# XuyangBai/D3Feat

Hardware: NVIDIA H100
Metric: points/sec through KPFCNN encoder (higher is better)
Workload: dtype f32

## Files before the change

### d3feat_b200/csrc/pool.cu

```cuda
#include "ops.cuh"

namespace d3f {

__global__ void __launch_bounds__(256) colmin_kernel(const float* __restrict__ x, int Ncap, const int* __restrict__ n_dev,
                                                     int C, unsigned* __restrict__ colmin_ord) {
  const int N = dyn_rows(Ncap, n_dev);
  __shared__ unsigned red[8][32];
  if (colmin_ord[C] != 0u) return;
  const int tx = threadIdx.x & 31, ty = threadIdx.x >> 5;
  const int c = blockIdx.x * 32 + tx;
  unsigned m = 0xffffffffu;
  if (c < C)
    for (int r = blockIdx.y * 8 + ty; r < N; r += gridDim.y * 8) m = min(m, f2ord(x[(size_t)r * C + c]));
  red[ty][tx] = m;
  __syncthreads();
  if (ty == 0 && c < C) {
#pragma unroll
    for (int k = 1; k < 8; ++k) m = min(m, red[k][tx]);
    atomicMin(&colmin_ord[c], m);
  }
}

template <int VEC>
__global__ void __launch_bounds__(256)
ind_max_pool_kernel(const float* __restrict__ x, const int* __restrict__ inds, int N1cap, int N2cap,
                    const int* __restrict__ n1_dev, const int* __restrict__ n2_dev, int H, int C, int slabs,
                    unsigned* __restrict__ colmin_ord, float* __restrict__ out) {
  const int N1 = dyn_rows(N1cap, n1_dev), N2 = dyn_rows(N2cap, n2_dev);
  const int gw = (blockIdx.x * blockDim.x + threadIdx.x) >> 5, lane = threadIdx.x & 31;
  const int warp = gw / slabs, slab = gw - warp * slabs;
  if (warp >= N2) return;
  const int* row = inds + (size_t)warp * H;
  const int c0 = slab * 32 * VEC + lane * VEC;
  if (c0 >= C) return;
  float best[VEC];
#pragma unroll
  for (int v = 0; v < VEC; ++v) best[v] = -3.402823466e38f;
  bool any_real = false;
  for (int h = 0; h < H; ++h) {
    int id = row[h];
    if (id < 0 || id >= N1) continue;
    any_real = true;
    const float* p = x + (size_t)id * C + c0;
    if (VEC == 4) {
      float4 t = *reinterpret_cast<const float4*>(p);
      best[0] = fmaxf(best[0], t.x); best[1 % VEC] = fmaxf(best[1 % VEC], t.y);
      best[2 % VEC] = fmaxf(best[2 % VEC], t.z); best[3 % VEC] = fmaxf(best[3 % VEC], t.w);
    } else {
      best[0] = fmaxf(best[0], *p);
    }
  }
  if (!any_real) {
    if (lane == 0 && slab == 0) colmin_ord[C] = 0u;
    return;
  }
  if (VEC == 4) {
    *reinterpret_cast<float4*>(out + (size_t)warp * C + c0) =
        make_float4(best[0], best[1 % VEC], best[2 % VEC], best[3 % VEC]);
  } else {
    out[(size_t)warp * C + c0] = best[0];
  }
}

__global__ void __launch_bounds__(256)
ind_max_pool_fix_kernel(const int* __restrict__ inds, int N1cap, int N2cap, const int* __restrict__ n1_dev,
                        const int* __restrict__ n2_dev, int H, int C, const unsigned* __restrict__ colmin_ord,
                        float* __restrict__ out) {
  if (colmin_ord[C] != 0u) return;
  const int N1 = dyn_rows(N1cap, n1_dev), N2 = dyn_rows(N2cap, n2_dev);
  const int lane = threadIdx.x & 31;
  for (int r = (blockIdx.x * blockDim.x + threadIdx.x) >> 5; r < N2; r += (gridDim.x * blockDim.x) >> 5) {
    bool real = false;
    for (int h = lane; h < H; h += 32) {
      int id = inds[(size_t)r * H + h];
      real = real || (id >= 0 && id < N1);
    }
    if (__any_sync(0xffffffffu, real)) continue;
    for (int c = lane; c < C; c += 32) out[(size_t)r * C + c] = ord2f(colmin_ord[c]);
  }
}

int ind_max_pool(const float* x, const int* inds, int N1, int N2, int H, int C, float* out, void* workspace,
                 size_t workspace_bytes, cudaStream_t stream, const int* n1_dev, const int* n2_dev) {
  D3F_REQUIRE(N1 >= 1 && N2 >= 0 && H >= 0 && C >= 1, D3F_ERR_INVALID, "ind_max_pool: bad shape N1=%d N2=%d H=%d C=%d",
              N1, N2, H, C);
  D3F_REQUIRE(workspace_bytes >= sizeof(unsigned) * ((size_t)C + 1), D3F_ERR_WORKSPACE,
              "ind_max_pool: workspace too small");
  if (N2 == 0) return D3F_OK;
  unsigned* colmin = (unsigned*)workspace;
  D3F_CUDA(cudaMemsetAsync(colmin, 0xff, sizeof(unsigned) * ((size_t)C + 1), stream));
  int blocks = ceil_div(N2 * 32, 256);
  bool v4 = (C % 4 == 0) && ((reinterpret_cast<uintptr_t>(x) & 15) == 0) && ((reinterpret_cast<uintptr_t>(out) & 15) == 0);
  const int slabs = ceil_div(C, v4 ? 128 : 32);
  const long long pool_blocks = ((long long)N2 * slabs * 32 + 255) / 256;
  D3F_REQUIRE(pool_blocks < (1ll << 31), D3F_ERR_CAPACITY, "ind_max_pool: %d rows x %d channels exceed the launch grid", N2, C);
  if (v4) ind_max_pool_kernel<4><<<(unsigned)pool_blocks, 256, 0, stream>>>(x, inds, N1, N2, n1_dev, n2_dev, H, C, slabs, colmin, out);
  else ind_max_pool_kernel<1><<<(unsigned)pool_blocks, 256, 0, stream>>>(x, inds, N1, N2, n1_dev, n2_dev, H, C, slabs, colmin, out);
  D3F_LAUNCH_CHECK("ind_max_pool_kernel");
  dim3 grid(ceil_div(C, 32), min(ceil_div(N1, 64), 4 * kNumSMs));
  colmin_kernel<<<grid, 256, 0, stream>>>(x, N1, n1_dev, C, colmin);
  D3F_LAUNCH_CHECK("colmin_kernel");
  ind_max_pool_fix_kernel<<<min(blocks, 4 * kNumSMs), 256, 0, stream>>>(inds, N1, N2, n1_dev, n2_dev, H, C, colmin, out);
  D3F_LAUNCH_CHECK("ind_max_pool_fix_kernel");
  return D3F_OK;
}

__global__ void __launch_bounds__(256)
closest_pool_kernel(const float* __restrict__ x, const int* __restrict__ inds, int N1cap, int N2cap,
                    const int* __restrict__ n1_dev, const int* __restrict__ n2_dev, int ld, int C,
                    float* __restrict__ out) {
  const int N1 = dyn_rows(N1cap, n1_dev), N2 = dyn_rows(N2cap, n2_dev);
  const int warp = (blockIdx.x * blockDim.x + threadIdx.x) >> 5, lane = threadIdx.x & 31;
  if (warp >= N2) return;
  int id = inds[(size_t)warp * ld];
  bool shadow = id < 0 || id >= N1;
  for (int c = lane; c < C; c += 32) out[(size_t)warp * C + c] = shadow ? 0.f : x[(size_t)id * C + c];
}

int closest_pool(const float* x, const int* inds, int N1, int N2, int ld_inds, int C, float* out, cudaStream_t stream,
                 const int* n1_dev, const int* n2_dev) {
  D3F_REQUIRE(N1 >= 0 && N2 >= 0 && ld_inds >= 1 && C >= 1, D3F_ERR_INVALID, "closest_pool: bad shape");
  if (N2 == 0) return D3F_OK;
  closest_pool_kernel<<<ceil_div(N2 * 32, 256), 256, 0, stream>>>(x, inds, N1, N2, n1_dev, n2_dev, ld_inds, C, out);
  D3F_LAUNCH_CHECK("closest_pool_kernel");
  return D3F_OK;
}

__global__ void __launch_bounds__(256) l2_normalize_kernel(const float* __restrict__ x, int Ncap,
                                                           const int* __restrict__ n_dev, int C, float eps,
                                                           float* __restrict__ out) {
  const int N = dyn_rows(Ncap, n_dev);
  const int warp = (blockIdx.x * blockDim.x + threadIdx.x) >> 5, lane = threadIdx.x & 31;
  if (warp >= N) return;
  float s = 0.f;
  for (int c = lane; c < C; c += 32) {
    float v = x[(size_t)warp * C + c];
    s = fmaf(v, v, s);
  }
#pragma unroll
  for (int o = 16; o > 0; o >>= 1) s += __shfl_xor_sync(0xffffffffu, s, o);
  float inv = rsqrtf(fmaxf(s, eps));
  float m = fmaxf(s, eps);
  inv = inv * (1.5f - 0.5f * m * inv * inv);
  for (int c = lane; c < C; c += 32) out[(size_t)warp * C + c] = x[(size_t)warp * C + c] * inv;
}

int l2_normalize(const float* x, int N, int C, float eps, float* out, cudaStream_t stream, const int* n_dev) {
  D3F_REQUIRE(N >= 0 && C >= 1, D3F_ERR_INVALID, "l2_normalize: bad shape");
  if (N == 0) return D3F_OK;
  l2_normalize_kernel<<<ceil_div(N * 32, 256), 256, 0, stream>>>(x, N, n_dev, C, eps, out);
  D3F_LAUNCH_CHECK("l2_normalize_kernel");
  return D3F_OK;
}

__global__ void __launch_bounds__(256)
cloud_max_kernel(const float* __restrict__ x, int Ncap, const int* __restrict__ n_dev, int D,
                 const int* __restrict__ start, int B, unsigned* __restrict__ cloud_max_ord,
                 unsigned char* __restrict__ nonzero) {
  const int N = dyn_rows(Ncap, n_dev);
  const int warp = (blockIdx.x * blockDim.x + threadIdx.x) >> 5, lane = threadIdx.x & 31;
  if (warp >= N) return;
  float m = -3.402823466e38f, s = 0.f;
  for (int c = lane; c < D; c += 32) {
    float v = x[(size_t)warp * D + c];
    m = fmaxf(m, v);
    s += v;
  }
#pragma unroll
  for (int o = 16; o > 0; o >>= 1) {
    m = fmaxf(m, __shfl_xor_sync(0xffffffffu, m, o));
    s += __shfl_xor_sync(0xffffffffu, s, o);
  }
  if (lane == 0) {
    if (warp < start[B]) atomicMax(&cloud_max_ord[batch_of(start, B, warp)], f2ord(m));
    nonzero[warp] = s != 0.f ? 1 : 0;
  }
}

__global__ void __launch_bounds__(256)
detection_score_kernel(const float* __restrict__ x, const int* __restrict__ nb, int Ncap,
                       const int* __restrict__ n_dev, int H, int D, const int* __restrict__ start, int B,
                       const unsigned* __restrict__ cloud_max_ord, const unsigned char* __restrict__ nonzero,
                       float* __restrict__ score) {
  const int N = dyn_rows(Ncap, n_dev);
  const int warp = (blockIdx.x * blockDim.x + threadIdx.x) >> 5, lane = threadIdx.x & 31;
  if (warp >= N) return;
  const float inv = warp < start[B] ? 1.f / (ord2f(cloud_max_ord[batch_of(start, B, warp)]) + 1e-6f) : 0.f;
  const int* row = nb + (size_t)warp * H;
  int cnt = 0;
  for (int h = 0; h < H; ++h) {
    int id = row[h];
    if (id >= 0 && id < N && nonzero[id]) ++cnt;
  }
  const float inv_cnt = 1.f / (float)max(cnt, 1);
  float dmax = -3.402823466e38f;
  for (int c = lane; c < D; c += 32) dmax = fmaxf(dmax, x[(size_t)warp * D + c] * inv);
#pragma unroll
  for (int o = 16; o > 0; o >>= 1) dmax = fmaxf(dmax, __shfl_xor_sync(0xffffffffu, dmax, o));
  float best = -3.402823466e38f;
  for (int c = lane; c < D; c += 32) {
    const float f = x[(size_t)warp * D + c] * inv;
    float mean = 0.f;
    for (int h = 0; h < H; ++h) {
      int id = row[h];
      if (id >= 0 && id < N) mean += x[(size_t)id * D + c] * inv;
    }
    mean *= inv_cnt;
    const float d = f - mean;
    const float softplus = d > 20.f ? d : log1pf(expf(d));
    best = fmaxf(best, softplus * (f / (1e-6f + dmax)));
  }
#pragma unroll
  for (int o = 16; o > 0; o >>= 1) best = fmaxf(best, __shfl_xor_sync(0xffffffffu, best, o));
  if (lane == 0) score[warp] = best;
}

size_t detection_scores_workspace_bytes(int N, int B) {
  return align_up(sizeof(int) * (size_t)(B + 1), 256) + align_up(sizeof(unsigned) * (size_t)B, 256) + align_up((size_t)N + 1, 256);
}

int detection_scores(const float* feats, const int* neighbors, const int* lengths, int B, int N, int H, int D,
                     float* out_scores, void* workspace, size_t workspace_bytes, cudaStream_t stream,
                     const int* n_dev) {
  D3F_REQUIRE(B >= 1 && B <= kMaxBatch && N >= 0 && H >= 0 && D >= 1, D3F_ERR_INVALID, "detection_scores: bad shape");
  D3F_REQUIRE(workspace_bytes >= detection_scores_workspace_bytes(N, B), D3F_ERR_WORKSPACE, "detection_scores: workspace too small");
  if (N == 0) return D3F_OK;
  Carver cv(workspace, workspace_bytes);
  int* start = cv.take<int>(B + 1);
  unsigned* cmax = cv.take<unsigned>(B);
  unsigned char* nonzero = cv.take<unsigned char>((size_t)N + 1);
  int rc = launch_batch_start(lengths, B, start, stream);
  if (rc) return rc;
  D3F_CUDA(cudaMemsetAsync(cmax, 0, sizeof(unsigned) * B, stream));
  cloud_max_kernel<<<ceil_div(N * 32, 256), 256, 0, stream>>>(feats, N, n_dev, D, start, B, cmax, nonzero);
  D3F_LAUNCH_CHECK("cloud_max_kernel");
  detection_score_kernel<<<ceil_div(N * 32, 256), 256, 0, stream>>>(feats, neighbors, N, n_dev, H, D, start, B, cmax, nonzero, out_scores);
  D3F_LAUNCH_CHECK("detection_score_kernel");
  return D3F_OK;
}

__global__ void __launch_bounds__(256)
affine_leaky_kernel(const float* __restrict__ x, long long total_cap, const int* __restrict__ n_dev, int C,
                    const float* __restrict__ scale, const float* __restrict__ shift,
                    const float* __restrict__ residual, float alpha, float* __restrict__ out) {
  const long long total = n_dev ? min(total_cap, (long long)max(__ldg(n_dev), 0) * C) : total_cap;
  for (long long i = (long long)blockIdx.x * blockDim.x + threadIdx.x; i < total; i += (long long)gridDim.x * blockDim.x) {
    int c = (int)(i % C);
    float y = x[i];
    if (scale) y = fmaf(y, scale[c], shift[c]);
    if (residual) y += residual[i];
    if (alpha >= 0.f) y = y > 0.f ? y : y * alpha;
    out[i] = y;
  }
}

int affine_leaky(const float* x, int N, int C, const float* scale, const float* shift, const float* residual,
                 float alpha, float* out, cudaStream_t stream, const int* n_dev) {
  D3F_REQUIRE(N >= 0 && C >= 1 && (scale == nullptr) == (shift == nullptr), D3F_ERR_INVALID, "affine_leaky: bad arguments");
  long long total = (long long)N * C;
  if (total == 0) return D3F_OK;
  int blocks = (int)min((total + 255) / 256, (long long)kNumSMs * 16);
  affine_leaky_kernel<<<blocks, 256, 0, stream>>>(x, total, n_dev, C, scale, shift, residual, alpha, out);
  D3F_LAUNCH_CHECK("affine_leaky_kernel");
  return D3F_OK;
}

}
```

### d3feat_b200/csrc/tc_gemm.cu

```cuda
#include <cuda.h>
#include <cudaTypedefs.h>
#include <stdlib.h>

#include "ops.cuh"
#include "tc_common.cuh"

namespace d3f {

constexpr int kTcBM = 128;
constexpr int kTcBK = 32;
constexpr int kTcConsumerWarps = 8;
constexpr int kTcThreads = 32 * kTcConsumerWarps + 32;

__global__ void __launch_bounds__(256) pack_weight_kernel(const float* __restrict__ W, int K, int N, int Kpad,
                                                          int Npad, float* __restrict__ packed) {
  long long total = (long long)Npad * Kpad;
  for (long long i = (long long)blockIdx.x * blockDim.x + threadIdx.x; i < total; i += (long long)gridDim.x * blockDim.x) {
    int k = (int)(i / Npad), n = (int)(i % Npad);
    float x = (n < N && k < K) ? W[(size_t)k * N + n] : 0.f;
    float hi, lo;
    split_tf32(x, hi, lo);
    int kc = k >> 5, kl = k & 31;
    size_t slab = (size_t)kc * 2 * Npad * 32;
    size_t off = (size_t)n * 32 + (size_t)((((kl >> 2) ^ (n & 7)) << 2) | (kl & 3));
    packed[slab + off] = hi;
    packed[slab + (size_t)Npad * 32 + off] = lo;
  }
}

int tc_padded_k(int K) { return (K + kTcBK - 1) / kTcBK * kTcBK; }
int tc_block_n(int N) { return N > 64 ? 128 : (N > 32 ? 64 : 32); }
int tc_padded_n(int N) { int bn = tc_block_n(N); return (N + bn - 1) / bn * bn; }
size_t tc_packed_floats(int K, int N) { return 2 * (size_t)tc_padded_k(K) * tc_padded_n(N); }

int tc_pack_weight(const float* W, int K, int N, float* packed, cudaStream_t stream) {
  D3F_REQUIRE(K >= 1 && N >= 1 && W && packed, D3F_ERR_INVALID, "pack_weight: bad arguments");
  int Kpad = tc_padded_k(K), Npad = tc_padded_n(N);
  long long total = (long long)Npad * Kpad;
  int blocks = (int)min((total + 255) / 256, (long long)kNumSMs * 8);
  pack_weight_kernel<<<blocks, 256, 0, stream>>>(W, K, N, Kpad, Npad, packed);
  D3F_LAUNCH_CHECK("pack_weight_kernel");
  return D3F_OK;
}

template <int BN>
struct TcSmem {
  static constexpr int kCtasPerSm = BN >= 128 ? 1 : 2;
  static constexpr int kStages = BN >= 64 ? 3 : 4;
  static constexpr int kABytes = kTcBM * 128;
  static constexpr int kBBytes = BN * 128;
  static constexpr int kStageBytes = kABytes + 2 * kBBytes;
  static constexpr int kEpiWarpBytes = 1024 + 3 * BN * 4;
  static constexpr int kTotal = kStages * kStageBytes + 1024  + 256  + kTcConsumerWarps * kEpiWarpBytes;
  static_assert(kCtasPerSm * (kTotal + 1024) <= 233472, "shared memory of an H100 SM (228 KB, 1 KB reserved per CTA)");
};

template <int BN>
__global__ void __launch_bounds__(kTcThreads, TcSmem<BN>::kCtasPerSm)
tc_gemm_kernel(const __grid_constant__ CUtensorMap tmA, const __grid_constant__ CUtensorMap tmA2, int K1,
               const float* __restrict__ Bp, float* __restrict__ C, int Mcap, int N, int Kpad, int Npad,
               int chunks_per_split, Epilogue ep) {
  const int M = ep.m_dev ? min(Mcap, max(__ldg(ep.m_dev) - ep.m_off, 0)) : Mcap;
  const int ntn = Npad / BN;
  const int tiles = ceil_div(M, kTcBM) * ntn;
  if ((int)blockIdx.x >= tiles) return;
  extern __shared__ uint8_t smem_raw[];
  using S = TcSmem<BN>;
  constexpr int kStages = S::kStages;
  uint8_t* smem = (uint8_t*)(((uintptr_t)smem_raw + 1023) & ~(uintptr_t)1023);
  uint64_t* full = (uint64_t*)(smem + kStages * S::kStageBytes);
  uint64_t* empty = full + kStages;

  const int tid = threadIdx.x, warp = tid >> 5, lane = tid & 31;
  const int kt0 = blockIdx.z * chunks_per_split;
  const int nk = min(Kpad / kTcBK - kt0, chunks_per_split);
  float* Cz = C + (size_t)blockIdx.z * Mcap * N;

  if (tid == 0) {
    for (int s = 0; s < kStages; ++s) {
      mbar_init(smem_u32(&full[s]), 1);
      mbar_init(smem_u32(&empty[s]), kTcConsumerWarps);
    }
    asm volatile("fence.mbarrier_init.release.cluster;" ::: "memory");
  }
  __syncthreads();

  if (warp == kTcConsumerWarps) {
    if (lane == 0) {
      const int total = (tiles - (int)blockIdx.x + (int)gridDim.x - 1) / (int)gridDim.x * nk;
      int tile = (int)blockIdx.x, kt = 0;
      for (int g = 0; g < total; ++g) {
        const int s = g % kStages;
        mbar_wait(smem_u32(&empty[s]), ((uint32_t)(g / kStages) & 1u) ^ 1u);
        const uint32_t st = smem_u32(smem + s * S::kStageBytes);
        const uint32_t fb = smem_u32(&full[s]);
        const int m0 = (tile / ntn) * kTcBM, n0 = (tile % ntn) * BN;
        const int k0 = (kt0 + kt) * kTcBK;
        mbar_arrive_expect_tx(fb, (uint32_t)S::kStageBytes);
        if (k0 < K1)
          tma_load_2d(st, &tmA, k0, m0, fb);
        else
          tma_load_2d(st, &tmA2, k0 - K1, m0, fb);
        const float* slab = Bp + (size_t)(kt0 + kt) * 2 * Npad * 32 + (size_t)n0 * 32;
        tma_bulk_g2s(st + S::kABytes, slab, S::kBBytes, fb);
        tma_bulk_g2s(st + S::kABytes + S::kBBytes, slab + (size_t)Npad * 32, S::kBBytes, fb);
        if (++kt == nk) {
          kt = 0;
          tile += (int)gridDim.x;
        }
      }
    }
  } else {
    constexpr int R = BN / 2;
    const int cw = warp >> 2;
    const int wq = warp & 3;
    const int r0 = 64 * cw + 16 * wq + (lane >> 2);
    const uint32_t a_row = (uint32_t)r0 * 128u + (uint32_t)(lane & 3) * 4u, a_swz = (uint32_t)(r0 & 7);
    auto load_a = [&](float* x, uint32_t sa, int j) {
#pragma unroll
      for (int q = 0; q < 4; ++q)
        x[q] = lds32(sa + a_row + (uint32_t)(q & 1) * 1024u + ((((uint32_t)(2 * j + (q >> 1))) ^ a_swz) << 4));
    };
    float acc[R], sum[R];
    int g = 0;
    for (int t = (int)blockIdx.x; t < tiles; t += (int)gridDim.x) {
      const int m0 = (t / ntn) * kTcBM, n0 = (t % ntn) * BN;
#pragma unroll
      for (int j = 0; j < R; ++j) sum[j] = 0.f;
      for (int kt = 0; kt < nk; ++kt, ++g) {
        const int s = g % kStages;
        mbar_wait(smem_u32(&full[s]), (uint32_t)(g / kStages) & 1u);
        const uint32_t sa = smem_u32(smem + s * S::kStageBytes);
        const uint64_t b_hi = make_smem_desc(sa + S::kABytes), b_lo = make_smem_desc(sa + S::kABytes + S::kBBytes);
        float x[4];
        uint32_t ah[2][4], al[2][4];
        load_a(x, sa, 0);
#pragma unroll
        for (int j = 0; j < R; ++j) acc[j] = 0.f;
#pragma unroll
        for (int j = 0; j < kTcBK / 8; ++j) {
          uint32_t* h = ah[j & 1];
          uint32_t* l = al[j & 1];
#pragma unroll
          for (int q = 0; q < 4; ++q) {
            float hi, lo;
            split_tf32(x[q], hi, lo);
            h[q] = __float_as_uint(hi);
            l[q] = __float_as_uint(lo);
          }
          const uint64_t adv = (uint64_t)((j * 32) >> 4);
          wgmma_fence();
          wgmma_tf32_rs<BN>(acc, h, b_hi + adv);
          wgmma_tf32_rs<BN>(acc, l, b_hi + adv);
          wgmma_tf32_rs<BN>(acc, h, b_lo + adv);
          wgmma_commit();
          if (j + 1 < kTcBK / 8) load_a(x, sa, j + 1);
          wgmma_wait<1>();
        }
        wgmma_wait<0>();
        wgmma_reg_fence<R>(acc);
        __syncwarp();
        if (lane == 0) mbar_arrive(smem_u32(&empty[s]));
#pragma unroll
        for (int j = 0; j < R; ++j) sum[j] += acc[j];
      }
      const bool has_bn = ep.bn_scale != nullptr, has_bias = ep.bias != nullptr, has_res = ep.residual != nullptr;
      const bool has_leaky = ep.leaky_alpha >= 0.f;
      const bool vec = (N & 3) == 0 &&
                       ((reinterpret_cast<uintptr_t>(C) | reinterpret_cast<uintptr_t>(ep.residual)) & 15) == 0;
      const uint32_t st_tile = smem_u32(smem + kStages * S::kStageBytes + 256) + (uint32_t)warp * S::kEpiWarpBytes;
      const uint32_t st_par = st_tile + 1024u;
      if (t == (int)blockIdx.x || ntn > 1) {
        for (int c = lane; c < BN; c += 32) {
          const int n = n0 + c;
          if (has_bn) {
            sts32(st_par + 4u * c, n < N ? ep.bn_scale[n] : 0.f);
            sts32(st_par + 4u * (BN + c), n < N ? ep.bn_shift[n] : 0.f);
          }
          if (has_bias) sts32(st_par + 4u * (2 * BN + c), n < N ? ep.bias[n] : 0.f);
        }
      }
#pragma unroll
      for (int h = 0; h < 2; ++h) {
#pragma unroll
        for (int cg = 0; cg < BN / 32; ++cg) {
          {
            const uint32_t r = (uint32_t)(lane >> 2), tq = (uint32_t)(lane & 3);
            const uint32_t swz = ((r & 3u) << 1) ^ (r >> 2);
#pragma unroll
            for (int jj = 0; jj < 4; ++jj) {
              const int j = 4 * cg + jj;
              sts64(st_tile + r * 128u + (((uint32_t)(2 * jj) + (tq >> 1)) ^ swz) * 16u + (tq & 1u) * 8u,
                    sum[4 * j + 2 * h], sum[4 * j + 2 * h + 1]);
            }
          }
          __syncwarp();
          const int pc = lane & 7;
          const int gn = n0 + 32 * cg + 4 * pc;
          const uint32_t par = st_par + 4u * (32 * cg + 4 * pc);
#pragma unroll
          for (int i = 0; i < 2; ++i) {
            const uint32_t r = (uint32_t)(lane >> 3) + 4u * i;
            const float4 v = lds128(st_tile + r * 128u + (((uint32_t)pc ^ ((r & 3u) << 1) ^ (r >> 2)) << 4));
            const int gm = m0 + 64 * cw + 16 * wq + 8 * h + (int)r;
            if (gm >= M || gn >= N) continue;
            const float rs = ep.rowscale != nullptr ? ep.rowscale[gm] : 1.f;
            const size_t orow = ep.row_map ? (size_t)ep.row_map[gm] : (size_t)gm;
            float* cp = Cz + orow * N + gn;
            const float* rp = has_res ? ep.residual + orow * N + gn : nullptr;
            float y[4] = {v.x * rs, v.y * rs, v.z * rs, v.w * rs};
            float res[4] = {0.f, 0.f, 0.f, 0.f};
            if (has_res) {
              if (vec) {
                const float4 rv = *reinterpret_cast<const float4*>(rp);
                res[0] = rv.x; res[1] = rv.y; res[2] = rv.z; res[3] = rv.w;
              } else {
#pragma unroll
                for (int e = 0; e < 4; ++e)
                  if (gn + e < N) res[e] = rp[e];
              }
            }
            if (has_bn) {
              const float4 sc = lds128(par), sh = lds128(par + 4u * BN);
              y[0] = fmaf(y[0], sc.x, sh.x); y[1] = fmaf(y[1], sc.y, sh.y);
              y[2] = fmaf(y[2], sc.z, sh.z); y[3] = fmaf(y[3], sc.w, sh.w);
            }
            if (has_bias) {
              const float4 bi = lds128(par + 8u * BN);
              y[0] += bi.x; y[1] += bi.y; y[2] += bi.z; y[3] += bi.w;
            }
#pragma unroll
            for (int e = 0; e < 4; ++e) {
              y[e] += res[e];
              if (has_leaky) y[e] = y[e] > 0.f ? y[e] : y[e] * ep.leaky_alpha;
            }
            if (vec) {
              *reinterpret_cast<float4*>(cp) = make_float4(y[0], y[1], y[2], y[3]);
            } else {
#pragma unroll
              for (int e = 0; e < 4; ++e)
                if (gn + e < N) cp[e] = y[e];
            }
          }
          __syncwarp();
        }
      }
    }
  }
}

__global__ void __launch_bounds__(256) splitk_reduce_kernel(const float* __restrict__ part, int splits, int Mcap, int N,
                                                            Epilogue ep, float* __restrict__ C) {
  const int M = ep.m_dev ? min(Mcap, max(__ldg(ep.m_dev) - ep.m_off, 0)) : Mcap;
  const long long slab = (long long)Mcap * N;
  long long total = (long long)M * N;
  for (long long i = (long long)blockIdx.x * blockDim.x + threadIdx.x; i < total; i += (long long)gridDim.x * blockDim.x) {
    int m = (int)(i / N), n = (int)(i % N);
    float y = 0.f;
    for (int z = 0; z < splits; ++z) y += part[(size_t)z * slab + i];
    if (ep.rowscale) y *= ep.rowscale[m];
    if (ep.bn_scale) y = fmaf(y, ep.bn_scale[n], ep.bn_shift[n]);
    if (ep.bias) y += ep.bias[n];
    const size_t orow = ep.row_map ? (size_t)ep.row_map[m] : (size_t)m;
    if (ep.residual) y += ep.residual[orow * N + n];
    if (ep.leaky_alpha >= 0.f) y = y > 0.f ? y : y * ep.leaky_alpha;
    C[orow * N + n] = y;
  }
}

static int encode_a_map(CUtensorMap* map, const float* A, int rows, int cols) {
  static PFN_cuTensorMapEncodeTiled_v12000 encode = nullptr;
  if (encode == nullptr) {
    void* fn = nullptr;
    cudaDriverEntryPointQueryResult q;
    D3F_CUDA(cudaGetDriverEntryPoint("cuTensorMapEncodeTiled", &fn, cudaEnableDefault, &q));
    D3F_REQUIRE(q == cudaDriverEntryPointSuccess && fn != nullptr, D3F_ERR_CUDA,
                "tc_gemm: the driver has no cuTensorMapEncodeTiled");
    encode = reinterpret_cast<PFN_cuTensorMapEncodeTiled_v12000>(fn);
  }
  const cuuint64_t dims[2] = {(cuuint64_t)cols, (cuuint64_t)rows};
  const cuuint64_t strides[1] = {(cuuint64_t)cols * sizeof(float)};
  const cuuint32_t box[2] = {(cuuint32_t)kTcBK, (cuuint32_t)kTcBM};
  const cuuint32_t elem[2] = {1, 1};
  const CUresult r = encode(map, CU_TENSOR_MAP_DATA_TYPE_FLOAT32, 2, const_cast<float*>(A), dims, strides, box, elem,
                            CU_TENSOR_MAP_INTERLEAVE_NONE, CU_TENSOR_MAP_SWIZZLE_128B, CU_TENSOR_MAP_L2_PROMOTION_L2_256B,
                            CU_TENSOR_MAP_FLOAT_OOB_FILL_NONE);
  D3F_REQUIRE(r == CUDA_SUCCESS, D3F_ERR_CUDA, "tc_gemm: cuTensorMapEncodeTiled failed (%d)", (int)r);
  return D3F_OK;
}

template <int BN>
static int launch_tc(const float* A, const float* A2, int K1, const float* Bp, float* C, int M, int N, int K,
                     const Epilogue& ep, cudaStream_t stream, int splits, float* split_ws, bool persistent) {
  using S = TcSmem<BN>;
  static bool configured = false;
  if (!configured) {
    D3F_CUDA(cudaFuncSetAttribute(tc_gemm_kernel<BN>, cudaFuncAttributeMaxDynamicSharedMemorySize, S::kTotal));
    configured = true;
  }
  const int Kpad = tc_padded_k(K), Npad = tc_padded_n(N);
  const int nk = Kpad / kTcBK;
  const int tiles = ceil_div(M, kTcBM) * (Npad / BN);
  CUtensorMap tmA, tmA2;
  if (A2 != nullptr) {
    int rc = encode_a_map(&tmA, A, M, K1);
    if (rc == D3F_OK) rc = encode_a_map(&tmA2, A2, M, K - K1);
    if (rc != D3F_OK) return rc;
  } else {
    const int rc = encode_a_map(&tmA, A, M, K);
    if (rc != D3F_OK) return rc;
    tmA2 = tmA;
    K1 = Kpad;
  }
  if (splits <= 1) {
    const int cap = kNumSMs * S::kCtasPerSm;
    const int grid = persistent && tiles > cap ? cap : tiles;
    tc_gemm_kernel<BN><<<grid, kTcThreads, S::kTotal, stream>>>(tmA, tmA2, K1, Bp, C, M, N, Kpad, Npad, nk, ep);
    D3F_LAUNCH_CHECK("tc_gemm_kernel");
    return D3F_OK;
  }
  const int cps = ceil_div(nk, splits);
  splits = ceil_div(nk, cps);
  Epilogue raw;
  raw.rowscale = nullptr; raw.bn_scale = nullptr; raw.bn_shift = nullptr; raw.bias = nullptr; raw.residual = nullptr;
  raw.leaky_alpha = -1.f; raw.row_map = nullptr; raw.m_dev = ep.m_dev; raw.m_off = ep.m_off;
  dim3 grid(tiles, 1, splits);
  tc_gemm_kernel<BN><<<grid, kTcThreads, S::kTotal, stream>>>(tmA, tmA2, K1, Bp, split_ws, M, N, Kpad, Npad, cps, raw);
  D3F_LAUNCH_CHECK("tc_gemm_kernel");
  long long total = (long long)M * N;
  int blocks = (int)min((total + 255) / 256, (long long)kNumSMs * 8);
  splitk_reduce_kernel<<<blocks, 256, 0, stream>>>(split_ws, splits, M, N, ep, C);
  D3F_LAUNCH_CHECK("splitk_reduce_kernel");
  return D3F_OK;
}

static int env_int(const char* name, int dflt) {
  const char* v = getenv(name);
  return v ? atoi(v) : dflt;
}

bool tc_gemm_supported(const float* A, int K) {
  return (K % 4 == 0) && ((reinterpret_cast<uintptr_t>(A) & 15) == 0);
}

int tc_gemm_splits(int M, int N, int K) {
  const int bn = tc_block_n(N);
  const long long ctas = (long long)ceil_div(M, kTcBM) * (tc_padded_n(N) / bn);
  const int nk = tc_padded_k(K) / kTcBK;
  if (ctas >= 96 || nk < 16) return 1;
  int best = 1;
  long long best_cost = (long long)ceil_div((int)ctas, kNumSMs) * nk * 8;
  for (int s = 2; s <= 8 && s <= nk / 4; ++s) {
    const int cps = ceil_div(nk, s);
    const int eff = ceil_div(nk, cps);
    if (eff != s) continue;
    long long cost = (long long)ceil_div((int)(ctas * s), kNumSMs) * cps * 8 + 40 + 6 * s;
    if (cost < best_cost) {
      best_cost = cost;
      best = s;
    }
  }
  return best;
}
size_t tc_gemm_split_ws_floats(int M, int N, int K) {
  const int bn = tc_block_n(N);
  const long long ctas = (long long)ceil_div(M, kTcBM) * (tc_padded_n(N) / bn);
  const int nk = tc_padded_k(K) / kTcBK;
  if (nk < 16) return 0;
  const long long tiles = ctas < 95 ? ctas : 95;
  return (size_t)(8 * tiles * kTcBM * bn);
}

int tc_gemm(const float* A, const float* Bp, float* C, int M, int N, int K, const Epilogue& ep, cudaStream_t stream,
            float* split_ws, const float* A2, int K1) {
  if (M <= 0 || N <= 0) return D3F_OK;
  D3F_REQUIRE(tc_gemm_supported(A, K), D3F_ERR_INVALID, "tc_gemm: needs K %% 4 == 0 and 16-byte aligned A");
  if (A2 != nullptr)
    D3F_REQUIRE(K1 > 0 && K1 < K && K1 % kTcBK == 0 && tc_gemm_supported(A2, K - K1), D3F_ERR_INVALID,
                "tc_gemm: split A operand needs K1 %% %d == 0 and a 16-byte aligned second matrix", kTcBK);
  int bn = tc_block_n(N);
  if (bn == 128 && K <= 256 && M >= 8192) bn = 64;
  const int splits = split_ws != nullptr ? tc_gemm_splits(M, N, K) : 1;
  const bool persistent = splits <= 1 && (tc_padded_k(K) / kTcBK <= 4 || env_int("D3F_TC_STREAM", 0) != 0);
  switch (bn) {
    case 128: return launch_tc<128>(A, A2, K1, Bp, C, M, N, K, ep, stream, splits, split_ws, persistent);
    case 64: return launch_tc<64>(A, A2, K1, Bp, C, M, N, K, ep, stream, splits, split_ws, persistent);
    default: return launch_tc<32>(A, A2, K1, Bp, C, M, N, K, ep, stream, splits, split_ws, persistent);
  }
}

}
```

Measured before the change: 64.70 million.

## Batch neighbor index loads in max-pool via ballot compaction; stagger GEMM warpgroup start

The max-pool kernel now reads 32 neighbor indices per warp at once and compacts the valid ones into shared memory with a ballot. It then issues 8 independent feature loads at a time, replacing the serial per-index loop and raising memory-level parallelism. In the TF32 wgmma GEMM with BN=128, the second consumer warpgroup now waits on a named barrier during the first k-tile until the first warpgroup has issued some MMAs, staggering their start. The stagger is meant to reduce contention, but it adds a barrier that may serialize work.

Measured after the change: 65.19 million (median of 6 runs). About the same (+0.8%).

```diff
diff --git a/d3feat_b200/csrc/pool.cu b/d3feat_b200/csrc/pool.cu
--- a/d3feat_b200/csrc/pool.cu
+++ b/d3feat_b200/csrc/pool.cu
@@ -26,21 +26,19 @@
 ind_max_pool_kernel(const float* __restrict__ x, const int* __restrict__ inds, int N1cap, int N2cap,
                     const int* __restrict__ n1_dev, const int* __restrict__ n2_dev, int H, int C, int slabs,
                     unsigned* __restrict__ colmin_ord, float* __restrict__ out) {
+  __shared__ int real_ids[8][32];
   const int N1 = dyn_rows(N1cap, n1_dev), N2 = dyn_rows(N2cap, n2_dev);
   const int gw = (blockIdx.x * blockDim.x + threadIdx.x) >> 5, lane = threadIdx.x & 31;
   const int warp = gw / slabs, slab = gw - warp * slabs;
   if (warp >= N2) return;
   const int* row = inds + (size_t)warp * H;
   const int c0 = slab * 32 * VEC + lane * VEC;
-  if (c0 >= C) return;
+  const bool active = c0 < C;
+  int* ids = real_ids[threadIdx.x >> 5];
   float best[VEC];
 #pragma unroll
   for (int v = 0; v < VEC; ++v) best[v] = -3.402823466e38f;
-  bool any_real = false;
-  for (int h = 0; h < H; ++h) {
-    int id = row[h];
-    if (id < 0 || id >= N1) continue;
-    any_real = true;
+  auto take = [&](int id) {
     const float* p = x + (size_t)id * C + c0;
     if (VEC == 4) {
       float4 t = *reinterpret_cast<const float4*>(p);
@@ -49,7 +47,44 @@
     } else {
       best[0] = fmaxf(best[0], *p);
     }
-  }
+  };
+  bool any_real = false;
+  for (int h0 = 0; h0 < H; h0 += 32) {
+    const int id = h0 + lane < H ? __ldg(row + h0 + lane) : -1;
+    const bool real = id >= 0 && id < N1;
+    const unsigned m = __ballot_sync(0xffffffffu, real);
+    if (real) ids[__popc(m & ((1u << lane) - 1u))] = id;
+    __syncwarp();
+    const int nr = __popc(m);
+    any_real = any_real || nr > 0;
+    if (active) {
+      int j = 0;
+      for (; j + 8 <= nr; j += 8) {
+        int r[8];
+#pragma unroll
+        for (int u = 0; u < 8; ++u) r[u] = ids[j + u];
+        if (VEC == 4) {
+          float4 t[8];
+#pragma unroll
+          for (int u = 0; u < 8; ++u) t[u] = *reinterpret_cast<const float4*>(x + (size_t)r[u] * C + c0);
+#pragma unroll
+          for (int u = 0; u < 8; ++u) {
+            best[0] = fmaxf(best[0], t[u].x); best[1 % VEC] = fmaxf(best[1 % VEC], t[u].y);
+            best[2 % VEC] = fmaxf(best[2 % VEC], t[u].z); best[3 % VEC] = fmaxf(best[3 % VEC], t[u].w);
+          }
+        } else {
+          float t[8];
+#pragma unroll
+          for (int u = 0; u < 8; ++u) t[u] = x[(size_t)r[u] * C + c0];
+#pragma unroll
+          for (int u = 0; u < 8; ++u) best[0] = fmaxf(best[0], t[u]);
+        }
+      }
+      for (; j < nr; ++j) take(ids[j]);
+    }
+    __syncwarp();
+  }
+  if (!active) return;
   if (!any_real) {
     if (lane == 0 && slab == 0) colmin_ord[C] = 0u;
     return;
diff --git a/d3feat_b200/csrc/tc_gemm.cu b/d3feat_b200/csrc/tc_gemm.cu
--- a/d3feat_b200/csrc/tc_gemm.cu
+++ b/d3feat_b200/csrc/tc_gemm.cu
@@ -134,6 +134,7 @@
         const uint64_t b_hi = make_smem_desc(sa + S::kABytes), b_lo = make_smem_desc(sa + S::kABytes + S::kBBytes);
         float x[4];
         uint32_t ah[2][4], al[2][4];
+        if (BN == 128 && g == 0 && cw == 1) asm volatile("bar.sync 2, %0;" ::"n"(32 * kTcConsumerWarps) : "memory");
         load_a(x, sa, 0);
 #pragma unroll
         for (int j = 0; j < R; ++j) acc[j] = 0.f;
@@ -155,6 +156,8 @@
           wgmma_tf32_rs<BN>(acc, h, b_lo + adv);
           wgmma_commit();
           if (j + 1 < kTcBK / 8) load_a(x, sa, j + 1);
+          if (BN == 128 && g == 0 && cw == 0 && j == 1)
+            asm volatile("bar.arrive 2, %0;" ::"n"(32 * kTcConsumerWarps) : "memory");
           wgmma_wait<1>();
         }
         wgmma_wait<0>();
```
